# qqueing/DeepSpeaker-pytorch

Hardware: NVIDIA H100
Metric: speaker-embeddings/sec (64-fbank x 160-frame -> 512-d) (higher is better)
Workload: dtype fp16

## Files before the change

deepspeaker_pytorch_b200/csrc/conv3x3_halo.cuh:

```cuda
#pragma once
#include "conv_umma.cuh"

namespace dsk {

constexpr int kHaloMaxBoxes = 25;
constexpr int kHaloMaxStages = 4;

struct HaloParams {
  int W, H, N;
  int q_begin;
  int tiles_m, tiles_c;
  int chunks;
  int cout;
  int a_stage_bytes;
  int a_stages, b_stages;
  int stg_bufs, res_bufs;
  int nboxes;
  int plane_positions;
  int8_t box_plane[kHaloMaxBoxes];
  int8_t box_first[kHaloMaxBoxes];
  int8_t box_last[kHaloMaxBoxes];
  int8_t box_ntaps[kHaloMaxBoxes];
  int16_t box_wtap[kHaloMaxBoxes];
  int16_t tap_shift[kHaloMaxBoxes][3];
  int out_planar;
  uint16_t* out_ptr;
  int out_plane_positions;
  int out_C;
  int flags;
  float clip_hi;
  float scale_c[512];
  float bias_c[512];
  int plain3x3;
  int late_trigger;
  int b_resident;
  unsigned pitch_magic, img_magic;
  int stream_k;
  int sk_q, sk_r;
  float* sk_partial;
  int* sk_flags;
  const uint16_t* res_ptr;
  long long* trace;
};

#define DSK_TRACE(role, idx)                                                                  \
  do {                                                                                        \
    if (p.trace && blockIdx.x == 0 && (idx) < 512) p.trace[(role) * 512 + (idx)] = clock64(); \
  } while (0)

template <int KIND, int TPB>
// ... 41 lines not shown
               "r"(smem_u32(smem_src)), "r"(c0), "r"(c1)
               : "memory");
}

constexpr int kHaloThreads = 384;
constexpr int halo_threads(int ew) { return 128 + 32 * ew; }

template <int N_TILE, bool BF16, int EW = 8, bool SK = false, int KIND = 1>
__global__ void __launch_bounds__(128 + 32 * EW, EW == 4 ? 2 : 1)
conv3x3_halo_kernel(const __grid_constant__ CUtensorMap tmIn, const __grid_constant__ CUtensorMap tmW,
                    const __grid_constant__ CUtensorMap tmOut, const __grid_constant__ CUtensorMap tmRes,
                    const HaloParams p) {
  using S = HaloSmem<N_TILE, EW>;
  constexpr int kEpiThreads = 32 * EW;
  constexpr int kCG = EW / 4;
  static_assert(!(EW == 4 && N_TILE == 256), "the two-CTA-per-SM shape runs 64- and 128-channel tiles");
  constexpr int kMW = 1;
  constexpr int kTM = S::kTileRows;
  const int kAStages = p.a_stages, kBStages = p.b_stages;
  constexpr int kChunksOut = N_TILE / 64;

  extern __shared__ uint8_t smem_raw[];
  uint8_t* smem = reinterpret_cast<uint8_t*>((reinterpret_cast<uintptr_t>(smem_raw) + 1023) & ~uintptr_t(1023));
  uint8_t* smem_a = smem;
  uint8_t* smem_b = smem_a + kAStages * p.a_stage_bytes;
  uint8_t* smem_stg = smem_b + kBStages * S::kBStageBytes;
  uint64_t* bars = reinterpret_cast<uint64_t*>(smem_stg + (p.stg_bufs + p.res_bufs) * kATileBytes);
  uint64_t* a_full = bars;
  uint64_t* a_empty = a_full + kHaloMaxStages;
  uint64_t* b_full = a_empty + kHaloMaxStages;
  uint64_t* b_empty = b_full + kHaloMaxStages;
// ... 95 lines not shown
          DSK_TRACE(0, 0);
        }
        __syncwarp();
      }
    }
  }
  if (warp == 1 && lane == 0) tma_prefetch_desc(&tmOut);
  __syncthreads();
  if (threadIdx.x == 0) DSK_TRACE(0, 481);
  pdl_wait();
  if (threadIdx.x == 0) DSK_TRACE(0, 482);

  if (warp == 0) {
    int as = 0, bs = 0;
    uint32_t aph = 0, bph = 0;
    bool first = true;
    int tcount = 1;
    bool a_pre = true;
    int cur = seg_begin();
    int tile, ub, ue;
    while (next_seg(cur, tile, ub, ue)) {
      int c0, q0;
      decode(tile, c0, q0);
      for (int u = ub; u < ue; ++u) {
        const int ch = u / p.nboxes, b = u - ch * p.nboxes;
        if (p.box_first[b] || u == ub) {
          if (a_pre) {
            a_pre = false;
          } else {
            mbar_wait(&a_empty[as], aph ^ 1);
            if (elect_one_sync()) {
              mbar_arrive_expect_tx(&a_full[as], halo_rows * 128);
              tma_load_2d(smem_a + as * p.a_stage_bytes, &tmIn, &a_full[as], ch * 64,
                          p.box_plane[b] * p.plane_positions + q0 - (p.W + 2));
              DSK_TRACE(0, tcount);
              ++tcount;
            }
            __syncwarp();
          }
          if (++as == kAStages) {
            as = 0;
            aph ^= 1;
          }
        }
        if (!p.b_resident || first) {
          if (pre_b > 0) {
            --pre_b;
          } else {
            mbar_wait(&b_empty[bs], bph ^ 1);
            if (elect_one_sync()) {
              mbar_arrive_expect_tx(&b_full[bs], S::kBStageBytes);
              tma_load_3d(smem_b + bs * S::kBStageBytes, &tmW, &b_full[bs], ch * 64, c0, p.box_wtap[b]);
            }
            __syncwarp();
          }
          if (++bs == kBStages) {
            bs = 0;
            bph ^= 1;
          }
        }
      }
      first = false;
    }
  } else if (warp >= 4) {
    const int cg = (warp >> 2) - 1;
    const int etid = threadIdx.x - 128;
    const bool wg_leader = (threadIdx.x & 127) == 0;
    const int fr = frag_row(), fc = frag_col();
    const bool has_res = (p.flags & CONV_RESIDUAL) != 0;
    const bool do_clip = (p.flags & CONV_CLIP) != 0;
    const int rows_real_end = p.N * (p.H + 1) + 1;
    const uint32_t clip_hi2 = pack2<BF16>(p.clip_hi, p.clip_hi);
    float acc[kMW][N_TILE / 2];
    int as = 0, bs = 0;
    uint32_t aph = 0, bph = 0;
    bool first = true;
    int buf = 0;
    int ecount = 0;
    int cur = seg_begin();
    int tile, ub, ue;
    int pend_b = -1, pend_a = -1;
    auto release_pending = [&]() {
      if (wg_leader) {
        if (pend_b >= 0) mbar_arrive(&b_empty[pend_b]);
        if (pend_a >= 0) mbar_arrive(&a_empty[pend_a]);
      }
      pend_b = pend_a = -1;
    };
    auto mma_box = [&](uint64_t da0, uint64_t db0, int ntaps_, const int16_t* shifts, bool zero) {
      wgmma_fence();
#pragma unroll
      for (int m = 0; m < kMW; ++m) {
        const uint64_t dam = da0 + static_cast<uint64_t>(cg * kMW + m) * kDescRows64;
        for (int t = 0; t < ntaps_; ++t) {
          const uint64_t da = dam + static_cast<uint64_t>(shifts[t]) * kDescRow;
#pragma unroll
          for (int k = 0; k < 4; ++k)
            wgmma_f16<N_TILE, BF16>(acc[m], da + 2 * k, db0 + (t * (N_TILE * 8) + 2 * k), (t > 0 || k > 0 || !zero) ? 1u : 0u);
        }
      }
      wgmma_commit();
    };
    while (next_seg(cur, tile, ub, ue)) {
      int c0, q0;
      decode(tile, c0, q0);
      {
        constexpr bool kResident = N_TILE == 64 && KIND == 1 && !S::kSmall;
        bool resident = false;
        if constexpr (kResident) resident = p.b_resident != 0;
        if (resident) {
          mbar_wait(&a_full[as], aph);
          if (first)
            for (int b = 0; b < 3; ++b) mbar_wait(&b_full[b], 0);
          const uint64_t da0 = gmma_desc_sw128(smem_u32(smem_a + as * p.a_stage_bytes));
          const uint64_t db0 = gmma_desc_sw128(smem_u32(smem_b));
          wgmma_fence();
#pragma unroll
          for (int m = 0; m < kMW; ++m) {
            const uint64_t dam = da0 + static_cast<uint64_t>(cg * kMW + m) * kDescRows64;
#pragma unroll
            for (int b = 0; b < 3; ++b)
#pragma unroll
              for (int t = 0; t < 3; ++t)
#pragma unroll
                for (int k = 0; k < 4; ++k)
                  wgmma_f16<N_TILE, BF16>(acc[m], dam + static_cast<uint64_t>(b * pitch + t) * kDescRow + 2 * k,
                                          db0 + ((b * 3 + t) * (N_TILE * 8) + 2 * k), (b > 0 || t > 0 || k > 0) ? 1u : 0u);
          }
          wgmma_commit();
          wgmma_wait<0>();
          if (wg_leader) mbar_arrive(&a_empty[as]);
          if (++as == kAStages) {
            as = 0;
            aph ^= 1;
          }
        } else {
          using Plan = HaloPlan<KIND, S::kTapsPerBox>;
          for (int ch = ub / Plan::kBoxes; ch * Plan::kBoxes < ue; ++ch) {
            uint64_t da0 = 0;
#pragma unroll
            for (int b = 0; b < Plan::kBoxes; ++b) {
              const int u = ch * Plan::kBoxes + b;
              if (u < ub || u >= ue) continue;
              if (Plan::first(b) || u == ub) {
                mbar_wait(&a_full[as], aph);
                da0 = gmma_desc_sw128(smem_u32(smem_a + as * p.a_stage_bytes));
              }
              mbar_wait(&b_full[bs], bph);
              const bool rel_a = Plan::last(b) || u == ue - 1;
              int16_t shifts[3];
#pragma unroll
              for (int t = 0; t < Plan::ntaps(b); ++t) shifts[t] = static_cast<int16_t>(Plan::row_i(b, t) * pitch + Plan::col_j(b, t));
              mma_box(da0, gmma_desc_sw128(smem_u32(smem_b + bs * S::kBStageBytes)), Plan::ntaps(b), shifts, u == ub);
              wgmma_wait<1>();
              release_pending();
              pend_b = bs;
              pend_a = rel_a ? as : -1;
              if (++bs == kBStages) {
                bs = 0;
                bph ^= 1;
              }
              if (rel_a) {
                if (++as == kAStages) {
                  as = 0;
                  aph ^= 1;
                }
              }
            }
          }
          wgmma_wait<0>();
          release_pending();
        }
        first = false;
#pragma unroll
        for (int m = 0; m < kMW; ++m) wgmma_fence_acc(acc[m]);
      }
      auto sk_slot = [&](int cta, int m, int i) -> float* {
        return p.sk_partial + (static_cast<size_t>(cta) * (kMW * N_TILE / 2) + m * (N_TILE / 2) + i) * kEpiThreads + etid;
      };
      if (SK && ub > 0) {
#pragma unroll
        for (int m = 0; m < kMW; ++m)
#pragma unroll
          for (int i = 0; i < N_TILE / 2; ++i) __stcg(sk_slot(blockIdx.x, m, i), acc[m][i]);
        __threadfence();
        named_bar_sync(3, kEpiThreads);
        if (etid == 0) st_release_gpu(p.sk_flags + blockIdx.x, 1);
        continue;
// ... 107 lines not shown
          named_bar_sync(1, kEpiThreads);
          if (etid == 0) {
            tma_store_2d(&tmOut, stg, c0 + j * 64, q0);
            tma_store_commit();
          }
          if (p.stg_bufs == 2) buf ^= 1;
        }
      }
      if (etid == 0) DSK_TRACE(2, ecount * 8 + 7);
      ++ecount;
    }
    if (etid == 0) tma_store_wait_all<0>();
  }
}

}
```

deepspeaker_pytorch_b200/csrc/dsk_api.cu:

```cuda
#include <cuda.h>
#include <cuda_runtime.h>

#include <algorithm>
#include <array>
#include <cstdarg>
#include <cstdio>
#include <cstdlib>
#include <cmath>
#include <cstring>
#include <map>
#include <string>
#include <tuple>
#include <vector>

#include "../../include/dsk.h"
#include "aam_kernels.cuh"
#include "ge2e_kernels.cuh"
#include "conv_umma.cuh"
#include "conv3x3_halo.cuh"
#include "conv1_umma.cuh"
#include "fbank_kernels.cuh"
#include "vad_kernels.cuh"
#include "augment_kernels.cuh"
#include "cluster_kernels.cuh"
// ... 711 lines not shown
  if (scale_d) CUDA_TRY(cudaMemcpy(sc->data(), scale_d, n * sizeof(float), cudaMemcpyDeviceToHost));
  if (bias_d) CUDA_TRY(cudaMemcpy(bi->data(), bias_d, n * sizeof(float), cudaMemcpyDeviceToHost));
  return DSK_OK;
}

int build_halo(const dsk_handle_s* h, HaloLaunch* L, const void* in, const void* wpk, const float* scale_host,
               const float* bias_host, const void* res, void* out, int N, int H, int W, int cin, int cout, int ksize,
               int flags, float clip_hi, int out_planar) {
  if (cin % 64 || cin < 64 || cout % 64 || cout < 64 || cout > 512)
    return fail(DSK_ERR_INVALID, "halo conv: channel counts must be multiples of 64 (got %d -> %d)", cin, cout);
  if (ksize != 3 && ksize != 5) return fail(DSK_ERR_INVALID, "halo conv: ksize must be 3 or 5");
  if (ksize == 3 && cin != cout) return fail(DSK_ERR_INVALID, "halo conv: the 3x3 form needs cin == cout");
  if (W > 34) return fail(DSK_ERR_INVALID, "halo conv: W must be <= 34 (got %d)", W);
  if (out_planar && ((H & 1) || (W & 1))) return fail(DSK_ERR_INVALID, "halo conv: planar output needs even H, W");
  if (out_planar && ksize != 3) return fail(DSK_ERR_INVALID, "halo conv: planar output is written by the 3x3 form only");
  const bool bf = h->bf16;
  dsk::HaloParams& p = L->p;
  memset(&p, 0, sizeof(p));
  p.W = W; p.H = H; p.N = N;
  p.q_begin = W + 1;
  const long q_end = static_cast<long>(N) * (H + 1) * (W + 1);
  const int tiles_m_ = static_cast<int>((q_end - p.q_begin + 127) / 128);
  const int n_tile = cout == 64 ? 64 : (h->n256 && cout % 256 == 0 && tiles_m_ * (cout / 256) >= h->n256_min_tiles) ? 256 : 128;
  const bool small = h->small_cta && n_tile == 128;
  const int tm = small ? 64 : 128;
  p.tiles_m = static_cast<int>((q_end - p.q_begin + tm - 1) / tm);
  const int tpb = (n_tile == 256 || small) ? 1 : 3;
  L->n_tile = n_tile;
  L->ew = small ? 4 : 8;
  p.tiles_c = cout / n_tile;
  p.chunks = cin / 64;
  p.cout = cout;
  p.flags = flags;
  p.clip_hi = clip_hi;
  for (int i = 0; i < cout; ++i) {
    p.scale_c[i] = scale_host ? scale_host[i] : 1.0f;
    p.bias_c[i] = bias_host ? bias_host[i] : 0.0f;
  }
  p.trace = h->trace;
  p.late_trigger = h->late_trigger ? 1 : 0;
// ... 30 lines not shown
        p.box_first[nb] = t0 == 0;
        p.box_last[nb] = t0 + tpb >= cnt;
        p.box_ntaps[nb] = (int8_t)(cnt - t0 < tpb ? cnt - t0 : tpb);
        p.box_wtap[nb] = (int16_t)(slot + t0);
        for (int t = 0; t < p.box_ntaps[nb]; ++t) {
          const int rs = perm[slot + t0 + t];
          const int dh = ((rs / 5) - 2) >> 1, dw = ((rs % 5) - 2) >> 1;
          p.tap_shift[nb][t] = (int16_t)((dh + 1) * (W + 1) + dw + 1);
        }
      }
      slot += cnt;
    }
    p.nboxes = nb;
  }
  p.plain3x3 = ksize == 3 ? 1 : 2;
  p.b_resident = (p.chunks == 1 && p.tiles_c == 1 && p.nboxes <= 3 && n_tile == 64) ? 1 : 0;
  p.res_ptr = (flags & dsk::CONV_RESIDUAL) ? static_cast<const uint16_t*>(res) : nullptr;
  p.out_planar = out_planar;
  if (out_planar) {
    p.out_ptr = static_cast<uint16_t*>(out);
    p.out_plane_positions = static_cast<int>(padded_positions(N, H / 2, W / 2));
    p.out_C = cout;
  }
  {
    const int halo_rows = tm + 2 * W + 4;
    p.a_stage_bytes = (halo_rows * 128 + 1023) / 1024 * 1024;
    const int b_bytes = tpb * n_tile * 128;
    const int fixed = dsk::HaloSmem<128>::kFixedBytes;
    if (small) {
      const int limit = 232448 / 2 - 1024;
      p.a_stages = 2;
      p.stg_bufs = 1;
      p.res_bufs = 0;
      int nb = (limit - fixed - p.a_stages * p.a_stage_bytes - p.stg_bufs * 16384) / b_bytes;
      if (nb > dsk::kHaloMaxStages) nb = dsk::kHaloMaxStages;
      if (nb < 2) return fail(DSK_ERR_INVALID, "halo conv (two CTAs per SM): shared memory does not fit");
      p.b_stages = nb;
      L->smem = p.a_stages * p.a_stage_bytes + p.b_stages * b_bytes + p.stg_bufs * 16384 + fixed;
    } else {
      const int limit = 227 * 1024;
      p.a_stages = n_tile == 64 ? 3 : 2;
      p.stg_bufs = 2;
      p.res_bufs = 0;
      int nb = (limit - fixed - p.a_stages * p.a_stage_bytes - p.stg_bufs * 16384) / b_bytes;
      p.b_stages = nb > dsk::kHaloMaxStages ? dsk::kHaloMaxStages : nb;
      if (p.b_resident) p.b_stages = 3;
      if (p.b_stages < 2) return fail(DSK_ERR_INVALID, "halo conv: shared memory does not fit");
      L->smem = p.a_stages * p.a_stage_bytes + p.b_stages * b_bytes + p.stg_bufs * 16384 + fixed;
    }
  }
  const int num_tiles = p.tiles_m * p.tiles_c;
  const int slots = h->num_sms * (small ? 2 : 1);
  L->grid = num_tiles < slots ? num_tiles : slots;
  p.stream_k = 0;
  if (h->stream_k && !small && !p.b_resident && p.plain3x3 && n_tile != 64) {
    const long units = static_cast<long>(p.chunks) * p.nboxes;
    const long total = units * num_tiles;
    long g = total / 6;
    if (g > h->num_sms) g = h->num_sms;
    if (g < 1) g = 1;
    const long span_tiles = (num_tiles + L->grid - 1) / L->grid * units;
    const long span_sk = (total + g - 1) / g;
    if (span_sk * 105 < span_tiles * 100 && total < (1l << 28)) {
      if (!h->sk_partial) {
        dsk_handle_s* hh = const_cast<dsk_handle_s*>(h);
        const size_t nb = static_cast<size_t>(h->num_sms) * 128 * 256 * sizeof(float);
        if (cudaMalloc(reinterpret_cast<void**>(&hh->sk_partial), nb) != cudaSuccess ||
            cudaMalloc(reinterpret_cast<void**>(&hh->sk_flags), h->num_sms * sizeof(int)) != cudaSuccess ||
            cudaMemset(hh->sk_flags, 0, h->num_sms * sizeof(int)) != cudaSuccess) {
          cudaGetLastError();
          return fail(DSK_ERR_CUDA, "halo conv: stream-K workspace allocation failed");
        }
      }
      p.stream_k = 1;
      p.sk_q = static_cast<int>(total / g);
      p.sk_r = static_cast<int>(total % g);
      p.sk_partial = h->sk_partial;
      p.sk_flags = h->sk_flags;
      L->grid = static_cast<int>(g);
    }
  }
  const uint64_t in_pos = static_cast<uint64_t>(npos) * (ksize == 5 ? 4 : 1);
  uint64_t idims[2] = {(uint64_t)cin, in_pos};
  uint64_t istr[1] = {2ull * cin};
  uint32_t box_in[2] = {64, (uint32_t)(tm + 2 * W + 4)};
  int rc = make_tmap(&L->tmIn, bf, in, 2, idims, istr, box_in);
  if (rc) return rc;
  uint64_t wd[3] = {(uint64_t)cin, (uint64_t)cout, (uint64_t)ntaps_total};
  uint64_t ws[2] = {2ull * cin, 2ull * cin * cout};
  uint32_t wb[3] = {64, (uint32_t)n_tile, (uint32_t)tpb};
  rc = make_tmap(&L->tmW, bf, wpk, 3, wd, ws, wb);
  if (rc) return rc;
  uint64_t odims[2] = {(uint64_t)cout, (uint64_t)npos};
  uint64_t ostr[1] = {2ull * cout};
  uint32_t box_out[2] = {64, (uint32_t)tm};
  const void* res_ptr = (flags & dsk::CONV_RESIDUAL) ? res : (out_planar ? in : out);
  rc = make_tmap(&L->tmRes, bf, res_ptr, 2, odims, ostr, box_out);
  if (rc) return rc;
  return make_tmap(&L->tmOut, bf, out_planar ? res_ptr : out, 2, odims, ostr, box_out);
}

template <int N_TILE, bool BF16, int EW, bool SK, int KIND>
int launch_halo_t(const HaloLaunch& L, cudaStream_t s) {
  auto kern = dsk::conv3x3_halo_kernel<N_TILE, BF16, EW, SK, KIND>;
  if (int rc = ensure_smem_optin(reinterpret_cast<const void*>(kern), EW == 4 ? 232448 / 2 - 1024 : 227 * 1024)) return rc;
  CUDA_TRY(launch_pdl(kern, dim3(L.grid), dim3(dsk::halo_threads(EW)), L.smem, s, L.tmIn, L.tmW, L.tmOut, L.tmRes, L.p));
  return DSK_OK;
}

template <int N_TILE, int EW, bool SK>
// ... 2 lines not shown
  if (h->bf16) return k5 ? launch_halo_t<N_TILE, true, EW, SK, 2>(L, s) : launch_halo_t<N_TILE, true, EW, SK, 1>(L, s);
  return k5 ? launch_halo_t<N_TILE, false, EW, SK, 2>(L, s) : launch_halo_t<N_TILE, false, EW, SK, 1>(L, s);
}

int launch_halo(const dsk_handle_s* h, const HaloLaunch& L, cudaStream_t s) {
  if (L.p.plain3x3 != 1 && L.p.plain3x3 != 2) return fail(DSK_ERR_INVALID, "halo conv: unknown tap plan %d", L.p.plain3x3);
  if (L.ew == 4) {
    if (L.n_tile != 128 || L.p.stream_k) return fail(DSK_ERR_INVALID, "two-CTAs-per-SM halo conv: 128-channel whole tiles only");
    return launch_halo_v<128, 4, false>(h, L, s);
  }
  if (L.p.stream_k) {
    if (L.n_tile == 128) return launch_halo_v<128, 8, true>(h, L, s);
    if (L.n_tile == 256) return launch_halo_v<256, 8, true>(h, L, s);
    return fail(DSK_ERR_INVALID, "stream-K halo conv: 128- or 256-channel tiles only");
  }
  return L.n_tile == 64 ? launch_halo_v<64, 8, false>(h, L, s)
                        : L.n_tile == 128 ? launch_halo_v<128, 8, false>(h, L, s) : launch_halo_v<256, 8, false>(h, L, s);
}

int check_handle(dsk_handle h) {
  if (!h) return fail(DSK_ERR_INVALID, "null handle");
  CUDA_TRY(cudaSetDevice(h->device));
  return DSK_OK;
}

template <typename T>
int dev_alloc(T** p, size_t n) {
  CUDA_TRY(cudaMalloc(reinterpret_cast<void**>(p), n * sizeof(T)));
  return DSK_OK;
}

void act_shape(int i, int T, int& H, int& W, int& C) {
// ... 2872 lines not shown
```

deepspeaker_pytorch_b200/csrc/dsk_ptx.cuh:

```cuda
#pragma once
#include <cuda.h>
#include <cuda_runtime.h>
#include <cuda_fp16.h>
#include <cuda_bf16.h>
#include <stdint.h>

namespace dsk {

__device__ __forceinline__ uint32_t smem_u32(const void* p) {
  return static_cast<uint32_t>(__cvta_generic_to_shared(p));
}

__device__ __forceinline__ bool elect_one_sync() {
  uint32_t pred = 0;
  uint32_t laneid = 0;
  asm volatile(
      "{\n\t"
      ".reg .b32 %%rx;\n\t"
      ".reg .pred %%px;\n\t"
      "elect.sync %%rx|%%px, %2;\n\t"
      "@%%px mov.s32 %1, 1;\n\t"
      "mov.s32 %0, %%rx;\n\t"
      "}"
      : "+r"(laneid), "+r"(pred)
// ... 158 lines not shown
          "{%0, %1, %2, %3, %4, %5, %6, %7, %8, %9, %10, %11, %12, %13, %14, %15, %16, %17, %18, %19, %20, %21, %22, %23, %24, %25, %26, %27, %28, %29, %30, %31, %32, %33, %34, %35, %36, %37, %38, %39, %40, %41, %42, %43, %44, %45, %46, %47, %48, %49, %50, %51, %52, %53, %54, %55, %56, %57, %58, %59, %60, %61, %62, %63, %64, %65, %66, %67, %68, %69, %70, %71, %72, %73, %74, %75, %76, %77, %78, %79, %80, %81, %82, %83, %84, %85, %86, %87, %88, %89, %90, %91, %92, %93, %94, %95, %96, %97, %98, %99, %100, %101, %102, %103, %104, %105, %106, %107, %108, %109, %110, %111, %112, %113, %114, %115, %116, %117, %118, %119, %120, %121, %122, %123, %124, %125, %126, %127}, "
          "%128, %129, p, 1, 1, %131, %132;\n\t}"
          : "+f"(d[0]), "+f"(d[1]), "+f"(d[2]), "+f"(d[3]), "+f"(d[4]), "+f"(d[5]), "+f"(d[6]), "+f"(d[7]), "+f"(d[8]), "+f"(d[9]), "+f"(d[10]), "+f"(d[11]), "+f"(d[12]), "+f"(d[13]), "+f"(d[14]), "+f"(d[15]), "+f"(d[16]), "+f"(d[17]), "+f"(d[18]), "+f"(d[19]), "+f"(d[20]), "+f"(d[21]), "+f"(d[22]), "+f"(d[23]), "+f"(d[24]), "+f"(d[25]), "+f"(d[26]), "+f"(d[27]), "+f"(d[28]), "+f"(d[29]), "+f"(d[30]), "+f"(d[31]), "+f"(d[32]), "+f"(d[33]), "+f"(d[34]), "+f"(d[35]), "+f"(d[36]), "+f"(d[37]), "+f"(d[38]), "+f"(d[39]), "+f"(d[40]), "+f"(d[41]), "+f"(d[42]), "+f"(d[43]), "+f"(d[44]), "+f"(d[45]), "+f"(d[46]), "+f"(d[47]), "+f"(d[48]), "+f"(d[49]), "+f"(d[50]), "+f"(d[51]), "+f"(d[52]), "+f"(d[53]), "+f"(d[54]), "+f"(d[55]), "+f"(d[56]), "+f"(d[57]), "+f"(d[58]), "+f"(d[59]), "+f"(d[60]), "+f"(d[61]), "+f"(d[62]), "+f"(d[63]), "+f"(d[64]), "+f"(d[65]), "+f"(d[66]), "+f"(d[67]), "+f"(d[68]), "+f"(d[69]), "+f"(d[70]), "+f"(d[71]), "+f"(d[72]), "+f"(d[73]), "+f"(d[74]), "+f"(d[75]), "+f"(d[76]), "+f"(d[77]), "+f"(d[78]), "+f"(d[79]), "+f"(d[80]), "+f"(d[81]), "+f"(d[82]), "+f"(d[83]), "+f"(d[84]), "+f"(d[85]), "+f"(d[86]), "+f"(d[87]), "+f"(d[88]), "+f"(d[89]), "+f"(d[90]), "+f"(d[91]), "+f"(d[92]), "+f"(d[93]), "+f"(d[94]), "+f"(d[95]), "+f"(d[96]), "+f"(d[97]), "+f"(d[98]), "+f"(d[99]), "+f"(d[100]), "+f"(d[101]), "+f"(d[102]), "+f"(d[103]), "+f"(d[104]), "+f"(d[105]), "+f"(d[106]), "+f"(d[107]), "+f"(d[108]), "+f"(d[109]), "+f"(d[110]), "+f"(d[111]), "+f"(d[112]), "+f"(d[113]), "+f"(d[114]), "+f"(d[115]), "+f"(d[116]), "+f"(d[117]), "+f"(d[118]), "+f"(d[119]), "+f"(d[120]), "+f"(d[121]), "+f"(d[122]), "+f"(d[123]), "+f"(d[124]), "+f"(d[125]), "+f"(d[126]), "+f"(d[127])
          : "l"(da), "l"(db), "r"(scale_d), "n"(TA), "n"(TB));
  } else {
      asm volatile(
          "{\n\t.reg .pred p;\n\tsetp.ne.b32 p, %130, 0;\n\t"
          "wgmma.mma_async.sync.aligned.m64n256k16.f32.f16.f16 "
          "{%0, %1, %2, %3, %4, %5, %6, %7, %8, %9, %10, %11, %12, %13, %14, %15, %16, %17, %18, %19, %20, %21, %22, %23, %24, %25, %26, %27, %28, %29, %30, %31, %32, %33, %34, %35, %36, %37, %38, %39, %40, %41, %42, %43, %44, %45, %46, %47, %48, %49, %50, %51, %52, %53, %54, %55, %56, %57, %58, %59, %60, %61, %62, %63, %64, %65, %66, %67, %68, %69, %70, %71, %72, %73, %74, %75, %76, %77, %78, %79, %80, %81, %82, %83, %84, %85, %86, %87, %88, %89, %90, %91, %92, %93, %94, %95, %96, %97, %98, %99, %100, %101, %102, %103, %104, %105, %106, %107, %108, %109, %110, %111, %112, %113, %114, %115, %116, %117, %118, %119, %120, %121, %122, %123, %124, %125, %126, %127}, "
          "%128, %129, p, 1, 1, %131, %132;\n\t}"
          : "+f"(d[0]), "+f"(d[1]), "+f"(d[2]), "+f"(d[3]), "+f"(d[4]), "+f"(d[5]), "+f"(d[6]), "+f"(d[7]), "+f"(d[8]), "+f"(d[9]), "+f"(d[10]), "+f"(d[11]), "+f"(d[12]), "+f"(d[13]), "+f"(d[14]), "+f"(d[15]), "+f"(d[16]), "+f"(d[17]), "+f"(d[18]), "+f"(d[19]), "+f"(d[20]), "+f"(d[21]), "+f"(d[22]), "+f"(d[23]), "+f"(d[24]), "+f"(d[25]), "+f"(d[26]), "+f"(d[27]), "+f"(d[28]), "+f"(d[29]), "+f"(d[30]), "+f"(d[31]), "+f"(d[32]), "+f"(d[33]), "+f"(d[34]), "+f"(d[35]), "+f"(d[36]), "+f"(d[37]), "+f"(d[38]), "+f"(d[39]), "+f"(d[40]), "+f"(d[41]), "+f"(d[42]), "+f"(d[43]), "+f"(d[44]), "+f"(d[45]), "+f"(d[46]), "+f"(d[47]), "+f"(d[48]), "+f"(d[49]), "+f"(d[50]), "+f"(d[51]), "+f"(d[52]), "+f"(d[53]), "+f"(d[54]), "+f"(d[55]), "+f"(d[56]), "+f"(d[57]), "+f"(d[58]), "+f"(d[59]), "+f"(d[60]), "+f"(d[61]), "+f"(d[62]), "+f"(d[63]), "+f"(d[64]), "+f"(d[65]), "+f"(d[66]), "+f"(d[67]), "+f"(d[68]), "+f"(d[69]), "+f"(d[70]), "+f"(d[71]), "+f"(d[72]), "+f"(d[73]), "+f"(d[74]), "+f"(d[75]), "+f"(d[76]), "+f"(d[77]), "+f"(d[78]), "+f"(d[79]), "+f"(d[80]), "+f"(d[81]), "+f"(d[82]), "+f"(d[83]), "+f"(d[84]), "+f"(d[85]), "+f"(d[86]), "+f"(d[87]), "+f"(d[88]), "+f"(d[89]), "+f"(d[90]), "+f"(d[91]), "+f"(d[92]), "+f"(d[93]), "+f"(d[94]), "+f"(d[95]), "+f"(d[96]), "+f"(d[97]), "+f"(d[98]), "+f"(d[99]), "+f"(d[100]), "+f"(d[101]), "+f"(d[102]), "+f"(d[103]), "+f"(d[104]), "+f"(d[105]), "+f"(d[106]), "+f"(d[107]), "+f"(d[108]), "+f"(d[109]), "+f"(d[110]), "+f"(d[111]), "+f"(d[112]), "+f"(d[113]), "+f"(d[114]), "+f"(d[115]), "+f"(d[116]), "+f"(d[117]), "+f"(d[118]), "+f"(d[119]), "+f"(d[120]), "+f"(d[121]), "+f"(d[122]), "+f"(d[123]), "+f"(d[124]), "+f"(d[125]), "+f"(d[126]), "+f"(d[127])
          : "l"(da), "l"(db), "r"(scale_d), "n"(TA), "n"(TB));
  }
}

template <int N, bool BF16, int TA = 0, int TB = 0>
__device__ __forceinline__ void wgmma_f16(float (&d)[N / 2], uint64_t da, uint64_t db, uint32_t scale_d) {
  static_assert(N == 64 || N == 128 || N == 256, "wgmma N tile");
  if constexpr (N == 64) wgmma_m64n64<BF16, TA, TB>(d, da, db, scale_d);
  else if constexpr (N == 128) wgmma_m64n128<BF16, TA, TB>(d, da, db, scale_d);
  else wgmma_m64n256<BF16, TA, TB>(d, da, db, scale_d);
}

__device__ __forceinline__ uint64_t gmma_desc_sw128(uint32_t smem_addr) {
  uint64_t d = 0;
  d |= static_cast<uint64_t>((smem_addr & 0x3FFFF) >> 4);
  d |= static_cast<uint64_t>(1) << 16;
  d |= static_cast<uint64_t>(1024 >> 4) << 32;
  d |= static_cast<uint64_t>(1) << 62;
  return d;
}
constexpr uint64_t kDescRow = 128 >> 4;
constexpr uint64_t kDescRows64 = 64 * kDescRow;

__device__ __forceinline__ void named_bar_sync(int id, int nthreads) {
  asm volatile("bar.sync %0, %1;" ::"r"(id), "r"(nthreads) : "memory");
}

template <bool BF16>
__device__ __forceinline__ uint32_t pack2(float a, float b) {
  if constexpr (BF16) {
    __nv_bfloat162 v = __floats2bfloat162_rn(a, b);
    return *reinterpret_cast<uint32_t*>(&v);
  } else {
    __half2 v = __floats2half2_rn(a, b);
    return *reinterpret_cast<uint32_t*>(&v);
  }
}
template <bool BF16>
__device__ __forceinline__ uint32_t clip2(uint32_t v, uint32_t lo, uint32_t hi) {
  if constexpr (BF16) {
    __nv_bfloat162 x = *reinterpret_cast<__nv_bfloat162*>(&v);
// ... 1 lines not shown
    return *reinterpret_cast<uint32_t*>(&x);
  } else {
    __half2 x = *reinterpret_cast<__half2*>(&v);
    x = __hmin2(__hmax2(x, *reinterpret_cast<__half2*>(&lo)), *reinterpret_cast<__half2*>(&hi));
    return *reinterpret_cast<uint32_t*>(&x);
  }
}
__device__ __forceinline__ void sts128(uint32_t addr, const uint4& v) {
  asm volatile("st.shared.v4.b32 [%0], {%1, %2, %3, %4};" ::"r"(addr), "r"(v.x), "r"(v.y), "r"(v.z), "r"(v.w) : "memory");
}
__device__ __forceinline__ uint4 lds128(uint32_t addr) {
  uint4 v;
  asm volatile("ld.shared.v4.b32 {%0, %1, %2, %3}, [%4];" : "=r"(v.x), "=r"(v.y), "=r"(v.z), "=r"(v.w) : "r"(addr) : "memory");
  return v;
}

template <bool BF16>
__device__ __forceinline__ float2 unpack2(uint32_t u) {
  if constexpr (BF16) {
    __nv_bfloat162 v = *reinterpret_cast<__nv_bfloat162*>(&u);
    return __bfloat1622float2(v);
  } else {
    __half2 v = *reinterpret_cast<__half2*>(&u);
    return __half22float2(v);
  }
}
template <bool BF16>
__device__ __forceinline__ uint16_t to16(float a) {
  if constexpr (BF16) {
    __nv_bfloat16 v = __float2bfloat16_rn(a);
// ... 17 lines not shown
```

Baseline: 168,700.

## Add dedicated transposed 64-channel 3x3 halo conv kernel with resident weights

Adds a specialised kernel for 64-output-channel 3x3 convolutions. It swaps the GEMM roles so the 64 output channels form the M=64 wgmma dimension and 168 spatial positions per warpgroup form the N dimension (m64n168). All nine weight taps stay resident in shared memory, and each CTA handles 336 positions with a two-stage input pipeline. Epilogue writes go through stmatrix/ldmatrix transposes, with an optional residual prefetch by TMA. The old b_resident path inside the general kernel is removed, and 64-channel layers no longer use the generic N_TILE=64 path, which is meant to cut the per-instruction overhead of narrow N=64 wgmma calls.

New measurement: 179,600, median of 6. +6.5%, better.

```diff
diff --git a/deepspeaker_pytorch_b200/csrc/conv3x3_halo.cuh b/deepspeaker_pytorch_b200/csrc/conv3x3_halo.cuh
--- a/deepspeaker_pytorch_b200/csrc/conv3x3_halo.cuh
+++ b/deepspeaker_pytorch_b200/csrc/conv3x3_halo.cuh
@@ -33,7 +33,6 @@
   float bias_c[512];
   int plain3x3;
   int late_trigger;
-  int b_resident;
   unsigned pitch_magic, img_magic;
   int stream_k;
   int sk_q, sk_r;
@@ -105,7 +104,8 @@
   using S = HaloSmem<N_TILE, EW>;
   constexpr int kEpiThreads = 32 * EW;
   constexpr int kCG = EW / 4;
-  static_assert(!(EW == 4 && N_TILE == 256), "the two-CTA-per-SM shape runs 64- and 128-channel tiles");
+  static_assert(N_TILE == 128 || N_TILE == 256, "64 output channels run conv3x3_halo_t64_kernel");
+  static_assert(!(EW == 4 && N_TILE == 256), "the two-CTA-per-SM shape runs 128-channel tiles");
   constexpr int kMW = 1;
   constexpr int kTM = S::kTileRows;
   const int kAStages = p.a_stages, kBStages = p.b_stages;
@@ -231,7 +231,6 @@
   if (warp == 0) {
     int as = 0, bs = 0;
     uint32_t aph = 0, bph = 0;
-    bool first = true;
     int tcount = 1;
     bool a_pre = true;
     int cur = seg_begin();
@@ -260,24 +259,21 @@
             aph ^= 1;
           }
         }
-        if (!p.b_resident || first) {
-          if (pre_b > 0) {
-            --pre_b;
-          } else {
-            mbar_wait(&b_empty[bs], bph ^ 1);
-            if (elect_one_sync()) {
-              mbar_arrive_expect_tx(&b_full[bs], S::kBStageBytes);
-              tma_load_3d(smem_b + bs * S::kBStageBytes, &tmW, &b_full[bs], ch * 64, c0, p.box_wtap[b]);
-            }
-            __syncwarp();
-          }
-          if (++bs == kBStages) {
-            bs = 0;
-            bph ^= 1;
-          }
-        }
-      }
-      first = false;
+        if (pre_b > 0) {
+          --pre_b;
+        } else {
+          mbar_wait(&b_empty[bs], bph ^ 1);
+          if (elect_one_sync()) {
+            mbar_arrive_expect_tx(&b_full[bs], S::kBStageBytes);
+            tma_load_3d(smem_b + bs * S::kBStageBytes, &tmW, &b_full[bs], ch * 64, c0, p.box_wtap[b]);
+          }
+          __syncwarp();
+        }
+        if (++bs == kBStages) {
+          bs = 0;
+          bph ^= 1;
+        }
+      }
     }
   } else if (warp >= 4) {
     const int cg = (warp >> 2) - 1;
@@ -291,7 +287,6 @@
     float acc[kMW][N_TILE / 2];
     int as = 0, bs = 0;
     uint32_t aph = 0, bph = 0;
-    bool first = true;
     int buf = 0;
     int ecount = 0;
     int cur = seg_begin();
@@ -322,73 +317,41 @@
       int c0, q0;
       decode(tile, c0, q0);
       {
-        constexpr bool kResident = N_TILE == 64 && KIND == 1 && !S::kSmall;
-        bool resident = false;
-        if constexpr (kResident) resident = p.b_resident != 0;
-        if (resident) {
-          mbar_wait(&a_full[as], aph);
-          if (first)
-            for (int b = 0; b < 3; ++b) mbar_wait(&b_full[b], 0);
-          const uint64_t da0 = gmma_desc_sw128(smem_u32(smem_a + as * p.a_stage_bytes));
-          const uint64_t db0 = gmma_desc_sw128(smem_u32(smem_b));
-          wgmma_fence();
-#pragma unroll
-          for (int m = 0; m < kMW; ++m) {
-            const uint64_t dam = da0 + static_cast<uint64_t>(cg * kMW + m) * kDescRows64;
-#pragma unroll
-            for (int b = 0; b < 3; ++b)
-#pragma unroll
-              for (int t = 0; t < 3; ++t)
-#pragma unroll
-                for (int k = 0; k < 4; ++k)
-                  wgmma_f16<N_TILE, BF16>(acc[m], dam + static_cast<uint64_t>(b * pitch + t) * kDescRow + 2 * k,
-                                          db0 + ((b * 3 + t) * (N_TILE * 8) + 2 * k), (b > 0 || t > 0 || k > 0) ? 1u : 0u);
-          }
-          wgmma_commit();
-          wgmma_wait<0>();
-          if (wg_leader) mbar_arrive(&a_empty[as]);
-          if (++as == kAStages) {
-            as = 0;
-            aph ^= 1;
-          }
-        } else {
-          using Plan = HaloPlan<KIND, S::kTapsPerBox>;
-          for (int ch = ub / Plan::kBoxes; ch * Plan::kBoxes < ue; ++ch) {
-            uint64_t da0 = 0;
-#pragma unroll
-            for (int b = 0; b < Plan::kBoxes; ++b) {
-              const int u = ch * Plan::kBoxes + b;
-              if (u < ub || u >= ue) continue;
-              if (Plan::first(b) || u == ub) {
-                mbar_wait(&a_full[as], aph);
-                da0 = gmma_desc_sw128(smem_u32(smem_a + as * p.a_stage_bytes));
-              }
-              mbar_wait(&b_full[bs], bph);
-              const bool rel_a = Plan::last(b) || u == ue - 1;
-              int16_t shifts[3];
-#pragma unroll
-              for (int t = 0; t < Plan::ntaps(b); ++t) shifts[t] = static_cast<int16_t>(Plan::row_i(b, t) * pitch + Plan::col_j(b, t));
-              mma_box(da0, gmma_desc_sw128(smem_u32(smem_b + bs * S::kBStageBytes)), Plan::ntaps(b), shifts, u == ub);
-              wgmma_wait<1>();
-              release_pending();
-              pend_b = bs;
-              pend_a = rel_a ? as : -1;
-              if (++bs == kBStages) {
-                bs = 0;
-                bph ^= 1;
-              }
-              if (rel_a) {
-                if (++as == kAStages) {
-                  as = 0;
-                  aph ^= 1;
-                }
+        using Plan = HaloPlan<KIND, S::kTapsPerBox>;
+        for (int ch = ub / Plan::kBoxes; ch * Plan::kBoxes < ue; ++ch) {
+          uint64_t da0 = 0;
+#pragma unroll
+          for (int b = 0; b < Plan::kBoxes; ++b) {
+            const int u = ch * Plan::kBoxes + b;
+            if (u < ub || u >= ue) continue;
+            if (Plan::first(b) || u == ub) {
+              mbar_wait(&a_full[as], aph);
+              da0 = gmma_desc_sw128(smem_u32(smem_a + as * p.a_stage_bytes));
+            }
+            mbar_wait(&b_full[bs], bph);
+            const bool rel_a = Plan::last(b) || u == ue - 1;
+            int16_t shifts[3];
+#pragma unroll
+            for (int t = 0; t < Plan::ntaps(b); ++t) shifts[t] = static_cast<int16_t>(Plan::row_i(b, t) * pitch + Plan::col_j(b, t));
+            mma_box(da0, gmma_desc_sw128(smem_u32(smem_b + bs * S::kBStageBytes)), Plan::ntaps(b), shifts, u == ub);
+            wgmma_wait<1>();
+            release_pending();
+            pend_b = bs;
+            pend_a = rel_a ? as : -1;
+            if (++bs == kBStages) {
+              bs = 0;
+              bph ^= 1;
+            }
+            if (rel_a) {
+              if (++as == kAStages) {
+                as = 0;
+                aph ^= 1;
               }
             }
           }
-          wgmma_wait<0>();
-          release_pending();
-        }
-        first = false;
+        }
+        wgmma_wait<0>();
+        release_pending();
 #pragma unroll
         for (int m = 0; m < kMW; ++m) wgmma_fence_acc(acc[m]);
       }
@@ -526,4 +489,212 @@
   }
 }
 
+constexpr int kT64Cols = 168;
+constexpr int kT64TileRows = 2 * kT64Cols;
+constexpr int kT64WeightBytes = 9 * 64 * 128;
+constexpr int kT64StageBytes = kT64TileRows * 128;
+constexpr int kT64FixedBytes = 256 + 1024;
+__host__ __device__ constexpr int t64_halo_box_rows(int W) { return ((kT64TileRows + 2 * W + 4 + 1) / 2 + 7) / 8 * 8; }
+
+template <bool BF16>
+__global__ void __launch_bounds__(kHaloThreads, 1)
+conv3x3_halo_t64_kernel(const __grid_constant__ CUtensorMap tmIn, const __grid_constant__ CUtensorMap tmW,
+                        const __grid_constant__ CUtensorMap tmOut, const __grid_constant__ CUtensorMap tmRes,
+                        const HaloParams p) {
+  constexpr int kAStages = 2;
+  extern __shared__ uint8_t smem_raw[];
+  uint8_t* smem = reinterpret_cast<uint8_t*>((reinterpret_cast<uintptr_t>(smem_raw) + 1023) & ~uintptr_t(1023));
+  uint8_t* smem_w = smem;
+  uint8_t* smem_a = smem_w + kT64WeightBytes;
+  uint8_t* smem_stg = smem_a + kAStages * p.a_stage_bytes;
+  uint64_t* bars = reinterpret_cast<uint64_t*>(smem_stg + kT64StageBytes);
+  uint64_t* a_full = bars;
+  uint64_t* a_empty = a_full + kAStages;
+  uint64_t* w_full = a_empty + kAStages;
+  uint64_t* res_full = w_full + 1;
+
+  const int warp = threadIdx.x >> 5;
+  const int lane = threadIdx.x & 31;
+  if (!p.late_trigger) pdl_launch_dependents();
+  const int pitch = p.W + 1;
+  const int box_rows = p.a_stage_bytes / 256;
+  const int num_tiles = p.tiles_m;
+  const bool has_res = (p.flags & CONV_RESIDUAL) != 0;
+
+  if (threadIdx.x == 0) {
+    tma_prefetch_desc(&tmIn);
+    tma_prefetch_desc(&tmW);
+    for (int i = 0; i < kAStages; ++i) {
+      mbar_init(&a_full[i], 1);
+      mbar_init(&a_empty[i], 2);
+    }
+    mbar_init(w_full, 1);
+    mbar_init(&res_full[0], 1);
+    mbar_init(&res_full[1], 1);
+    fence_barrier_init();
+  }
+  __syncthreads();
+  if (warp == 0) {
+    if (elect_one_sync()) {
+      mbar_arrive_expect_tx(w_full, kT64WeightBytes);
+      for (int b = 0; b < 3; ++b) tma_load_3d(smem_w + b * (kT64WeightBytes / 3), &tmW, w_full, 0, 0, 3 * b);
+    }
+    __syncwarp();
+    pdl_wait();
+    int as = 0;
+    uint32_t aph = 0;
+    for (int tile = blockIdx.x, k = 0; tile < num_tiles; tile += gridDim.x, ++k) {
+      const int q0 = p.q_begin + tile * kT64TileRows;
+      if (k >= kAStages) mbar_wait(&a_empty[as], aph ^ 1);
+      if (elect_one_sync()) {
+        uint8_t* dst = smem_a + as * p.a_stage_bytes;
+        mbar_arrive_expect_tx(&a_full[as], p.a_stage_bytes);
+        tma_load_2d(dst, &tmIn, &a_full[as], 0, q0 - (p.W + 2));
+        tma_load_2d(dst + box_rows * 128, &tmIn, &a_full[as], 0, q0 - (p.W + 2) + box_rows);
+      }
+      __syncwarp();
+      if (++as == kAStages) {
+        as = 0;
+        aph ^= 1;
+      }
+    }
+  } else if (warp >= 4) {
+    pdl_wait();
+    const int cg = (warp >> 2) - 1;
+    const int wtid = threadIdx.x & 127;
+    const bool wg_leader = wtid == 0;
+    const int bar_id = 1 + cg;
+    const int fr = frag_row(), fc = frag_col();
+    const bool do_clip = (p.flags & CONV_CLIP) != 0;
+    const bool out_planar = p.out_planar != 0;
+    const int rows_real_end = p.N * (p.H + 1) + 1;
+    const uint32_t clip_hi2 = pack2<BF16>(p.clip_hi, p.clip_hi);
+    const float sc0 = p.scale_c[fr], bi0 = p.bias_c[fr], sc1 = p.scale_c[fr + 8], bi1 = p.bias_c[fr + 8];
+    const uint32_t stg_s = smem_u32(smem_stg);
+    uint8_t* my_stg = smem_stg + cg * kT64Cols * 128;
+    const int sm_row0 = cg * kT64Cols + (lane & 7);
+    const int sm_chunk = 2 * (warp & 3) + ((lane >> 3) & 1);
+    auto issue_res = [&](int tile) {
+      mbar_arrive_expect_tx(&res_full[cg], kT64Cols * 128);
+      tma_load_2d(my_stg, &tmRes, &res_full[cg], 0, p.q_begin + tile * kT64TileRows + cg * kT64Cols);
+    };
+    if (has_res && wg_leader && static_cast<int>(blockIdx.x) < num_tiles) issue_res(blockIdx.x);
+    float acc[kT64Cols / 2];
+    int as = 0;
+    uint32_t aph = 0, rph = 0;
+    bool first = true;
+    const uint64_t dw0 = gmma_desc_sw128(smem_u32(smem_w));
+    for (int tile = blockIdx.x; tile < num_tiles; tile += gridDim.x) {
+      const int q0 = p.q_begin + tile * kT64TileRows;
+      const bool last = tile + static_cast<int>(gridDim.x) >= num_tiles;
+      mbar_wait(&a_full[as], aph);
+      if (first) {
+        mbar_wait(w_full, 0);
+        if (cg == 1) named_bar_sync(3, 256);
+      }
+      const uint64_t db0 = gmma_desc_sw128(smem_u32(smem_a + as * p.a_stage_bytes)) + static_cast<uint64_t>(cg * kT64Cols) * kDescRow;
+      wgmma_fence();
+#pragma unroll
+      for (int r = 0; r < 3; ++r)
+#pragma unroll
+        for (int s = 0; s < 3; ++s)
+#pragma unroll
+          for (int k = 0; k < 4; ++k)
+            wgmma_f16<kT64Cols, BF16>(acc, dw0 + static_cast<uint64_t>(r * 3 + s) * kDescRows64 + 2 * k,
+                                      db0 + static_cast<uint64_t>(r * pitch + s) * kDescRow + 2 * k,
+                                      (r > 0 || s > 0 || k > 0) ? 1u : 0u);
+      wgmma_commit();
+      wgmma_wait<0>();
+      wgmma_fence_acc(acc);
+      if (first && cg == 0) named_bar_arrive(3, 256);
+      first = false;
+      if (wg_leader) mbar_arrive(&a_empty[as]);
+      if (++as == kAStages) {
+        as = 0;
+        aph ^= 1;
+      }
+      if (p.late_trigger && last) pdl_launch_dependents();
+      if (has_res) {
+        mbar_wait(&res_full[cg], rph);
+        rph ^= 1;
+      } else if (!out_planar) {
+        if (wg_leader) tma_store_wait_read<0>();
+        named_bar_sync(bar_id, 128);
+      }
+      int R, cc, rr;
+      {
+        const int q = q0 + cg * kT64Cols + fc;
+        R = static_cast<int>(__umulhi(static_cast<unsigned>(q), p.pitch_magic));
+        cc = q - R * pitch;
+        rr = R - static_cast<int>(__umulhi(static_cast<unsigned>(R), p.img_magic)) * (p.H + 1);
+      }
+#pragma unroll
+      for (int i = 0; i < kT64Cols / 8; ++i) {
+        const bool row_junk = rr == 0 || R >= rows_real_end;
+        const bool j0 = row_junk || cc == 0;
+        const bool j1 = (cc + 1 == pitch) || row_junk;
+        const uint32_t keep = (j0 ? 0u : 0x0000FFFFu) | (j1 ? 0u : 0xFFFF0000u);
+        const uint32_t addr = stg_s + sw128_off16(sm_row0 + 8 * i, 8 * sm_chunk);
+        uint32_t rv[2] = {0u, 0u};
+        if (has_res) ldsm_x2_trans(addr, rv[0], rv[1]);
+        uint32_t o[2];
+#pragma unroll
+        for (int h = 0; h < 2; ++h) {
+          float f0 = fmaf(acc[4 * i + 2 * h], h ? sc1 : sc0, h ? bi1 : bi0);
+          float f1 = fmaf(acc[4 * i + 2 * h + 1], h ? sc1 : sc0, h ? bi1 : bi0);
+          if (has_res) {
+            const float2 t = unpack2<BF16>(rv[h]);
+            f0 += t.x;
+            f1 += t.y;
+          }
+          o[h] = pack2<BF16>(f0, f1);
+          if (do_clip) o[h] = clip2<BF16>(o[h], 0u, clip_hi2);
+          o[h] &= keep;
+        }
+        stsm_x2_trans(addr, o[0], o[1]);
+        cc += 8;
+        while (cc >= pitch) {
+          cc -= pitch;
+          ++R;
+          if (++rr == p.H + 1) rr = 0;
+        }
+      }
+      if (!out_planar) {
+        fence_proxy_async_smem();
+        named_bar_sync(bar_id, 128);
+        if (wg_leader) {
+          tma_store_2d(&tmOut, my_stg, 0, q0 + cg * kT64Cols);
+          tma_store_commit();
+          if (has_res && !last) {
+            tma_store_wait_read<0>();
+            issue_res(tile + gridDim.x);
+          }
+        }
+      } else {
+        named_bar_sync(bar_id, 128);
+        const int H2 = p.H >> 1, W2 = p.W >> 1;
+        for (int piece = wtid; piece < kT64Cols * 8; piece += 128) {
+          const int row = cg * kT64Cols + (piece >> 3), k = piece & 7;
+          const int q = q0 + row;
+          const int Rq = static_cast<int>(__umulhi(static_cast<unsigned>(q), p.pitch_magic));
+          const int cq = q - Rq * pitch;
+          const int n = static_cast<int>(__umulhi(static_cast<unsigned>(Rq), p.img_magic));
+          const int hh = Rq - 1 - n * (p.H + 1), ww = cq - 1;
+          if (cq == 0 || hh < 0 || Rq >= rows_real_end) continue;
+          const long q2 = static_cast<long>(n * (H2 + 1) + (hh >> 1) + 1) * (W2 + 1) + (ww >> 1) + 1;
+          const long plane = (hh & 1) * 2 + (ww & 1);
+          const uint4 v = lds128(stg_s + row * 128 + (((k ^ row) & 7) << 4));
+          *reinterpret_cast<uint4*>(p.out_ptr + (plane * p.out_plane_positions + q2) * p.out_C + k * 8) = v;
+        }
+        named_bar_sync(bar_id, 128);
+        if (has_res && !last && wg_leader) {
+          fence_proxy_async_smem();
+          issue_res(tile + gridDim.x);
+        }
+      }
+    }
+    if (wg_leader) tma_store_wait_all<0>();
+  }
 }
+
+}
diff --git a/deepspeaker_pytorch_b200/csrc/dsk_api.cu b/deepspeaker_pytorch_b200/csrc/dsk_api.cu
--- a/deepspeaker_pytorch_b200/csrc/dsk_api.cu
+++ b/deepspeaker_pytorch_b200/csrc/dsk_api.cu
@@ -749,6 +749,7 @@
   if (W > 34) return fail(DSK_ERR_INVALID, "halo conv: W must be <= 34 (got %d)", W);
   if (out_planar && ((H & 1) || (W & 1))) return fail(DSK_ERR_INVALID, "halo conv: planar output needs even H, W");
   if (out_planar && ksize != 3) return fail(DSK_ERR_INVALID, "halo conv: planar output is written by the 3x3 form only");
+  if (cout == 64 && ksize != 3) return fail(DSK_ERR_INVALID, "halo conv: 64 output channels need the 3x3 form");
   const bool bf = h->bf16;
   dsk::HaloParams& p = L->p;
   memset(&p, 0, sizeof(p));
@@ -758,7 +759,8 @@
   const int tiles_m_ = static_cast<int>((q_end - p.q_begin + 127) / 128);
   const int n_tile = cout == 64 ? 64 : (h->n256 && cout % 256 == 0 && tiles_m_ * (cout / 256) >= h->n256_min_tiles) ? 256 : 128;
   const bool small = h->small_cta && n_tile == 128;
-  const int tm = small ? 64 : 128;
+  const bool t64 = n_tile == 64;
+  const int tm = t64 ? dsk::kT64TileRows : small ? 64 : 128;
   p.tiles_m = static_cast<int>((q_end - p.q_begin + tm - 1) / tm);
   const int tpb = (n_tile == 256 || small) ? 1 : 3;
   L->n_tile = n_tile;
@@ -819,7 +821,6 @@
     p.nboxes = nb;
   }
   p.plain3x3 = ksize == 3 ? 1 : 2;
-  p.b_resident = (p.chunks == 1 && p.tiles_c == 1 && p.nboxes <= 3 && n_tile == 64) ? 1 : 0;
   p.res_ptr = (flags & dsk::CONV_RESIDUAL) ? static_cast<const uint16_t*>(res) : nullptr;
   p.out_planar = out_planar;
   if (out_planar) {
@@ -827,7 +828,15 @@
     p.out_plane_positions = static_cast<int>(padded_positions(N, H / 2, W / 2));
     p.out_C = cout;
   }
-  {
+  uint32_t halo_box_rows = static_cast<uint32_t>(tm + 2 * W + 4);
+  if (t64) {
+    halo_box_rows = dsk::t64_halo_box_rows(W);
+    p.a_stage_bytes = 2 * halo_box_rows * 128;
+    p.a_stages = 2;
+    p.stg_bufs = 1;
+    L->smem = dsk::kT64WeightBytes + p.a_stages * p.a_stage_bytes + dsk::kT64StageBytes + dsk::kT64FixedBytes;
+    if (L->smem > 227 * 1024) return fail(DSK_ERR_INVALID, "halo conv: shared memory does not fit");
+  } else {
     const int halo_rows = tm + 2 * W + 4;
     p.a_stage_bytes = (halo_rows * 128 + 1023) / 1024 * 1024;
     const int b_bytes = tpb * n_tile * 128;
@@ -844,12 +853,11 @@
       L->smem = p.a_stages * p.a_stage_bytes + p.b_stages * b_bytes + p.stg_bufs * 16384 + fixed;
     } else {
       const int limit = 227 * 1024;
-      p.a_stages = n_tile == 64 ? 3 : 2;
+      p.a_stages = 2;
       p.stg_bufs = 2;
       p.res_bufs = 0;
       int nb = (limit - fixed - p.a_stages * p.a_stage_bytes - p.stg_bufs * 16384) / b_bytes;
       p.b_stages = nb > dsk::kHaloMaxStages ? dsk::kHaloMaxStages : nb;
-      if (p.b_resident) p.b_stages = 3;
       if (p.b_stages < 2) return fail(DSK_ERR_INVALID, "halo conv: shared memory does not fit");
       L->smem = p.a_stages * p.a_stage_bytes + p.b_stages * b_bytes + p.stg_bufs * 16384 + fixed;
     }
@@ -858,7 +866,7 @@
   const int slots = h->num_sms * (small ? 2 : 1);
   L->grid = num_tiles < slots ? num_tiles : slots;
   p.stream_k = 0;
-  if (h->stream_k && !small && !p.b_resident && p.plain3x3 && n_tile != 64) {
+  if (h->stream_k && !small && p.plain3x3 && !t64) {
     const long units = static_cast<long>(p.chunks) * p.nboxes;
     const long total = units * num_tiles;
     long g = total / 6;
@@ -888,7 +896,7 @@
   const uint64_t in_pos = static_cast<uint64_t>(npos) * (ksize == 5 ? 4 : 1);
   uint64_t idims[2] = {(uint64_t)cin, in_pos};
   uint64_t istr[1] = {2ull * cin};
-  uint32_t box_in[2] = {64, (uint32_t)(tm + 2 * W + 4)};
+  uint32_t box_in[2] = {64, halo_box_rows};
   int rc = make_tmap(&L->tmIn, bf, in, 2, idims, istr, box_in);
   if (rc) return rc;
   uint64_t wd[3] = {(uint64_t)cin, (uint64_t)cout, (uint64_t)ntaps_total};
@@ -898,7 +906,7 @@
   if (rc) return rc;
   uint64_t odims[2] = {(uint64_t)cout, (uint64_t)npos};
   uint64_t ostr[1] = {2ull * cout};
-  uint32_t box_out[2] = {64, (uint32_t)tm};
+  uint32_t box_out[2] = {64, (uint32_t)(t64 ? dsk::kT64Cols : tm)};
   const void* res_ptr = (flags & dsk::CONV_RESIDUAL) ? res : (out_planar ? in : out);
   rc = make_tmap(&L->tmRes, bf, res_ptr, 2, odims, ostr, box_out);
   if (rc) return rc;
@@ -931,8 +939,14 @@
     if (L.n_tile == 256) return launch_halo_v<256, 8, true>(h, L, s);
     return fail(DSK_ERR_INVALID, "stream-K halo conv: 128- or 256-channel tiles only");
   }
-  return L.n_tile == 64 ? launch_halo_v<64, 8, false>(h, L, s)
-                        : L.n_tile == 128 ? launch_halo_v<128, 8, false>(h, L, s) : launch_halo_v<256, 8, false>(h, L, s);
+  if (L.n_tile == 64) {
+    if (L.p.plain3x3 != 1) return fail(DSK_ERR_INVALID, "halo conv: 64 output channels need the 3x3 form");
+    auto kern = h->bf16 ? dsk::conv3x3_halo_t64_kernel<true> : dsk::conv3x3_halo_t64_kernel<false>;
+    if (int rc = ensure_smem_optin(reinterpret_cast<const void*>(kern), 227 * 1024)) return rc;
+    CUDA_TRY(launch_pdl(kern, dim3(L.grid), dim3(dsk::kHaloThreads), L.smem, s, L.tmIn, L.tmW, L.tmOut, L.tmRes, L.p));
+    return DSK_OK;
+  }
+  return L.n_tile == 128 ? launch_halo_v<128, 8, false>(h, L, s) : launch_halo_v<256, 8, false>(h, L, s);
 }
 
 int check_handle(dsk_handle h) {
diff --git a/deepspeaker_pytorch_b200/csrc/dsk_ptx.cuh b/deepspeaker_pytorch_b200/csrc/dsk_ptx.cuh
--- a/deepspeaker_pytorch_b200/csrc/dsk_ptx.cuh
+++ b/deepspeaker_pytorch_b200/csrc/dsk_ptx.cuh
@@ -196,11 +196,33 @@
   }
 }
 
+template <bool BF16, int TA, int TB>
+__device__ __forceinline__ void wgmma_m64n168(float (&d)[84], uint64_t da, uint64_t db, uint32_t scale_d) {
+  if constexpr (BF16) {
+      asm volatile(
+          "{\n\t.reg .pred p;\n\tsetp.ne.b32 p, %86, 0;\n\t"
+          "wgmma.mma_async.sync.aligned.m64n168k16.f32.bf16.bf16 "
+          "{%0, %1, %2, %3, %4, %5, %6, %7, %8, %9, %10, %11, %12, %13, %14, %15, %16, %17, %18, %19, %20, %21, %22, %23, %24, %25, %26, %27, %28, %29, %30, %31, %32, %33, %34, %35, %36, %37, %38, %39, %40, %41, %42, %43, %44, %45, %46, %47, %48, %49, %50, %51, %52, %53, %54, %55, %56, %57, %58, %59, %60, %61, %62, %63, %64, %65, %66, %67, %68, %69, %70, %71, %72, %73, %74, %75, %76, %77, %78, %79, %80, %81, %82, %83}, "
+          "%84, %85, p, 1, 1, %87, %88;\n\t}"
+          : "+f"(d[0]), "+f"(d[1]), "+f"(d[2]), "+f"(d[3]), "+f"(d[4]), "+f"(d[5]), "+f"(d[6]), "+f"(d[7]), "+f"(d[8]), "+f"(d[9]), "+f"(d[10]), "+f"(d[11]), "+f"(d[12]), "+f"(d[13]), "+f"(d[14]), "+f"(d[15]), "+f"(d[16]), "+f"(d[17]), "+f"(d[18]), "+f"(d[19]), "+f"(d[20]), "+f"(d[21]), "+f"(d[22]), "+f"(d[23]), "+f"(d[24]), "+f"(d[25]), "+f"(d[26]), "+f"(d[27]), "+f"(d[28]), "+f"(d[29]), "+f"(d[30]), "+f"(d[31]), "+f"(d[32]), "+f"(d[33]), "+f"(d[34]), "+f"(d[35]), "+f"(d[36]), "+f"(d[37]), "+f"(d[38]), "+f"(d[39]), "+f"(d[40]), "+f"(d[41]), "+f"(d[42]), "+f"(d[43]), "+f"(d[44]), "+f"(d[45]), "+f"(d[46]), "+f"(d[47]), "+f"(d[48]), "+f"(d[49]), "+f"(d[50]), "+f"(d[51]), "+f"(d[52]), "+f"(d[53]), "+f"(d[54]), "+f"(d[55]), "+f"(d[56]), "+f"(d[57]), "+f"(d[58]), "+f"(d[59]), "+f"(d[60]), "+f"(d[61]), "+f"(d[62]), "+f"(d[63]), "+f"(d[64]), "+f"(d[65]), "+f"(d[66]), "+f"(d[67]), "+f"(d[68]), "+f"(d[69]), "+f"(d[70]), "+f"(d[71]), "+f"(d[72]), "+f"(d[73]), "+f"(d[74]), "+f"(d[75]), "+f"(d[76]), "+f"(d[77]), "+f"(d[78]), "+f"(d[79]), "+f"(d[80]), "+f"(d[81]), "+f"(d[82]), "+f"(d[83])
+          : "l"(da), "l"(db), "r"(scale_d), "n"(TA), "n"(TB));
+  } else {
+      asm volatile(
+          "{\n\t.reg .pred p;\n\tsetp.ne.b32 p, %86, 0;\n\t"
+          "wgmma.mma_async.sync.aligned.m64n168k16.f32.f16.f16 "
+          "{%0, %1, %2, %3, %4, %5, %6, %7, %8, %9, %10, %11, %12, %13, %14, %15, %16, %17, %18, %19, %20, %21, %22, %23, %24, %25, %26, %27, %28, %29, %30, %31, %32, %33, %34, %35, %36, %37, %38, %39, %40, %41, %42, %43, %44, %45, %46, %47, %48, %49, %50, %51, %52, %53, %54, %55, %56, %57, %58, %59, %60, %61, %62, %63, %64, %65, %66, %67, %68, %69, %70, %71, %72, %73, %74, %75, %76, %77, %78, %79, %80, %81, %82, %83}, "
+          "%84, %85, p, 1, 1, %87, %88;\n\t}"
+          : "+f"(d[0]), "+f"(d[1]), "+f"(d[2]), "+f"(d[3]), "+f"(d[4]), "+f"(d[5]), "+f"(d[6]), "+f"(d[7]), "+f"(d[8]), "+f"(d[9]), "+f"(d[10]), "+f"(d[11]), "+f"(d[12]), "+f"(d[13]), "+f"(d[14]), "+f"(d[15]), "+f"(d[16]), "+f"(d[17]), "+f"(d[18]), "+f"(d[19]), "+f"(d[20]), "+f"(d[21]), "+f"(d[22]), "+f"(d[23]), "+f"(d[24]), "+f"(d[25]), "+f"(d[26]), "+f"(d[27]), "+f"(d[28]), "+f"(d[29]), "+f"(d[30]), "+f"(d[31]), "+f"(d[32]), "+f"(d[33]), "+f"(d[34]), "+f"(d[35]), "+f"(d[36]), "+f"(d[37]), "+f"(d[38]), "+f"(d[39]), "+f"(d[40]), "+f"(d[41]), "+f"(d[42]), "+f"(d[43]), "+f"(d[44]), "+f"(d[45]), "+f"(d[46]), "+f"(d[47]), "+f"(d[48]), "+f"(d[49]), "+f"(d[50]), "+f"(d[51]), "+f"(d[52]), "+f"(d[53]), "+f"(d[54]), "+f"(d[55]), "+f"(d[56]), "+f"(d[57]), "+f"(d[58]), "+f"(d[59]), "+f"(d[60]), "+f"(d[61]), "+f"(d[62]), "+f"(d[63]), "+f"(d[64]), "+f"(d[65]), "+f"(d[66]), "+f"(d[67]), "+f"(d[68]), "+f"(d[69]), "+f"(d[70]), "+f"(d[71]), "+f"(d[72]), "+f"(d[73]), "+f"(d[74]), "+f"(d[75]), "+f"(d[76]), "+f"(d[77]), "+f"(d[78]), "+f"(d[79]), "+f"(d[80]), "+f"(d[81]), "+f"(d[82]), "+f"(d[83])
+          : "l"(da), "l"(db), "r"(scale_d), "n"(TA), "n"(TB));
+  }
+}
+
 template <int N, bool BF16, int TA = 0, int TB = 0>
 __device__ __forceinline__ void wgmma_f16(float (&d)[N / 2], uint64_t da, uint64_t db, uint32_t scale_d) {
-  static_assert(N == 64 || N == 128 || N == 256, "wgmma N tile");
+  static_assert(N == 64 || N == 128 || N == 168 || N == 256, "wgmma N tile");
   if constexpr (N == 64) wgmma_m64n64<BF16, TA, TB>(d, da, db, scale_d);
   else if constexpr (N == 128) wgmma_m64n128<BF16, TA, TB>(d, da, db, scale_d);
+  else if constexpr (N == 168) wgmma_m64n168<BF16, TA, TB>(d, da, db, scale_d);
   else wgmma_m64n256<BF16, TA, TB>(d, da, db, scale_d);
 }
 
@@ -218,6 +240,9 @@
 __device__ __forceinline__ void named_bar_sync(int id, int nthreads) {
   asm volatile("bar.sync %0, %1;" ::"r"(id), "r"(nthreads) : "memory");
 }
+__device__ __forceinline__ void named_bar_arrive(int id, int nthreads) {
+  asm volatile("bar.arrive %0, %1;" ::"r"(id), "r"(nthreads) : "memory");
+}
 
 template <bool BF16>
 __device__ __forceinline__ uint32_t pack2(float a, float b) {
@@ -249,6 +274,12 @@
   asm volatile("ld.shared.v4.b32 {%0, %1, %2, %3}, [%4];" : "=r"(v.x), "=r"(v.y), "=r"(v.z), "=r"(v.w) : "r"(addr) : "memory");
   return v;
 }
+__device__ __forceinline__ void ldsm_x2_trans(uint32_t addr, uint32_t& r0, uint32_t& r1) {
+  asm volatile("ldmatrix.sync.aligned.m8n8.x2.trans.shared.b16 {%0, %1}, [%2];" : "=r"(r0), "=r"(r1) : "r"(addr) : "memory");
+}
+__device__ __forceinline__ void stsm_x2_trans(uint32_t addr, uint32_t r0, uint32_t r1) {
+  asm volatile("stmatrix.sync.aligned.m8n8.x2.trans.shared.b16 [%0], {%1, %2};" ::"r"(addr), "r"(r0), "r"(r1) : "memory");
+}
 
 template <bool BF16>
 __device__ __forceinline__ float2 unpack2(uint32_t u) {
```
